# leodd/Lifted-Hybrid-Variational-Inference

Measured on AMD Instinct MI355X. Metric: lbp_sweeps_per_sec_10M_edge_hybrid_mrf, higher is better.
Workload: dtype f64

## Files before the change

include/lhvi.h:

```cpp
#ifndef LHVI_H
#define LHVI_H

#include <stddef.h>
#include <stdint.h>

#ifdef __cplusplus
extern "C" {
#endif

#define LHVI_ABI_VERSION 17
#define LHVI_MAX_ARITY 6

#define LHVI_OK 0
#define LHVI_E_ARG (-1)
#define LHVI_E_LAUNCH (-2)
#define LHVI_E_UNSUPPORTED (-3)
#define LHVI_E_NODEVICE (-4)
#define LHVI_E_NOT_PD (-5)

#define LHVI_POT_GENERIC 0
#define LHVI_POT_TABLE 1
#define LHVI_POT_GAUSSIAN 2
#define LHVI_POT_QUADRATIC 3
#define LHVI_POT_HYBRID_QUADRATIC 4
#define LHVI_POT_LINEAR_GAUSSIAN 5
#define LHVI_POT_X2 6
#define LHVI_POT_XY 7
#define LHVI_POT_MLN 8
#define LHVI_POT_MLN_HARD 9
#define LHVI_POT_IMAGE_NODE 10
#define LHVI_POT_IMAGE_EDGE 11

typedef struct lhvi_graph {
// ... 127 lines not shown
    const void* cq_desc;
    int32_t n_cq;
    const int32_t* v2f_wide;
    int32_t n_v2f_wide;
    const int32_t* v2f_narrow;
    int32_t n_v2f_narrow;
    const int32_t* v2f_hub;
    int32_t n_v2f_hub;
    const int32_t* v2f_mid16;
    int32_t n_v2f_mid16;
    const int32_t* v2f_mid32;
    int32_t n_v2f_mid32;
    const int32_t* prop_hub;
    int32_t n_prop_hub;
    double* prop_partial;
    const int32_t* resample_vars;
    int32_t n_resample_vars;
    const void* small16_desc;
    int32_t n_small16;
    const void* small32_desc;
    int32_t n_small32;
    const int64_t* halo_off;
    double* halo_buf;
} lhvi_pbp_t;

#define LHVI_PBP_DESC_BYTES 128
#define LHVI_PBP_TICKET_WORDS 16
#define LHVI_PBP_TICKET_COUNTERS 8
int lhvi_pbp_describe(const lhvi_graph_t* g, const lhvi_pots_t* pots, const lhvi_pbp_t* s, const int32_t* edges, int32_t count,
                      void* desc_out, void* stream);
int lhvi_pbp_describe_cq(const lhvi_graph_t* g, const lhvi_pots_t* pots, const lhvi_pbp_t* s, const int32_t* edges, int32_t count,
                         void* desc_out, void* stream);
int lhvi_pbp_var_sum(const lhvi_graph_t* g, const lhvi_pbp_t* s, const double* f2v, double* out, void* stream);
int lhvi_pbp_domain_grid(const lhvi_graph_t* g, const lhvi_pbp_t* s, double* x, void* stream);
int lhvi_pbp_refine_grid(const lhvi_graph_t* g, const lhvi_pbp_t* s, const double* logb, double* x, double* best, double* best_val,
                         void* stream);
int lhvi_debug_exp(const double* x, double* y, int64_t n, void* stream);
int lhvi_debug_exp_acc(const double* x, const double* c, double* y, int64_t n, void* stream);
int lhvi_debug_exp_acc_floor(const double* x, const double* c, double* y, int64_t n, void* stream);
int lhvi_debug_log(const double* x, double* y, int64_t n, int32_t which, void* stream);

int lhvi_pbp_classify(const lhvi_graph_t* g, const lhvi_pots_t* pots, const lhvi_pbp_t* s, uint8_t* edge_class, void* stream);

int lhvi_pbp_uniq(const lhvi_graph_t* g, int32_t n, const double* particles, const int32_t* np, uint8_t* uniq, void* stream);
int lhvi_pbp_v2f(const lhvi_graph_t* g, const lhvi_pbp_t* s, const double* f2v, double* v2f, void* stream);
int lhvi_pbp_f2v(const lhvi_graph_t* g, const lhvi_pots_t* pots, const lhvi_pbp_t* s, const double* v2f, double* f2v, void* stream);
// ... 207 lines not shown
```

lifted-hybrid-variational-inference_amd/csrc/fastmath.hpp:

```cpp
#pragma once
#include "common.hpp"

namespace lhvi {

#include "exp_table.inc"
constexpr int EXP_TAB_N = 1 << LHVI_EXP_TABLE_BITS;

__device__ __forceinline__ double exp_core(double t, const double* __restrict__ tab ) {
    const double MAGIC = LHVI_SCONST(6755399441055744.0);
    const double u = fma(t, LHVI_SCONST(LHVI_EXP_INV_STEP), MAGIC);
    const int nn = __double2loint(u);
    const double kd = u - MAGIC;
    double r = fma(kd, LHVI_SCONST(-LHVI_EXP_STEP_HI), t);
    r = fma(kd, LHVI_SCONST(-LHVI_EXP_STEP_LO), r);
    double p = fma(r, LHVI_SCONST(1.6666666666666666667e-1), 0.5);
    p = fma(p, r, 1.0);
    p = fma(p, r, 1.0);
    return ldexp(tab[nn & (EXP_TAB_N - 1)] * p, nn >> LHVI_EXP_TABLE_BITS);
}

__device__ __forceinline__ void load_exp_table(double* __restrict__ tab) {
    for (int i = threadIdx.x; i < EXP_TAB_N; i += blockDim.x) tab[i] = EXP_TAB[i];
    __syncthreads();
}
// ... 10 lines not shown
    double p = fma(r, 1.6666666666666666667e-1, 0.5);
    p = fma(p, r, 1.0);
    o.scale = fma(p, r, 1.0);
    return o;
}

__device__ __forceinline__ double exp_accumulate(double acc, double t, double magic, const double* __restrict__ tab) {
    double u;
    asm("v_fma_f64 %0, %1, %2, %3" : "=v"(u) : "v"(t), "s"((double)LHVI_EXP_INV_STEP), "v"(magic));
    const int nn = __double2loint(u);
    const double kd = u - magic;
    const double r = fma(kd, -LHVI_EXP_STEP_HI, t);
    double p = fma(r, 1.6666666666666666667e-1, 0.5);
    p = fma(p, r, 1.0);
    p = fma(p, r, 1.0);
    return fma(ldexp(tab[nn & (EXP_TAB_N - 1)], nn >> LHVI_EXP_TABLE_BITS), p, acc);
}

struct ExpShiftFloor { double magic, scale; };

__device__ __forceinline__ void round_down_on() { asm volatile("s_setreg_imm32_b32 hwreg(HW_REG_MODE, 2, 2), 2\n\ts_nop 1" ::: "memory"); }
__device__ __forceinline__ void round_down_off() { asm volatile("s_setreg_imm32_b32 hwreg(HW_REG_MODE, 2, 2), 0\n\ts_nop 1" ::: "memory"); }

__device__ __forceinline__ ExpShiftFloor exp_shift_floor(double C) {
    const double MAGIC = 6755399441055744.0;
    ExpShiftFloor o;
    const double m = fma(C, LHVI_EXP_INV_STEP, MAGIC);
    const double kd = m - MAGIC;
    double r = fma(kd, -LHVI_EXP_STEP_HI, C);
    r = fma(kd, -LHVI_EXP_STEP_LO, r);
    double p = fma(r, 1.6666666666666666667e-1, 0.5);
    p = fma(p, r, 1.0);
    o.scale = fma(p, r, 1.0) * LHVI_EXPF_SCALE;
    o.magic = 844424930131968.0 + (kd - (double)(24 << LHVI_EXP_TABLE_BITS));
    return o;
}

__device__ __forceinline__ double exp_accumulate_floor(double acc, double s, double magic, const double* __restrict__ tab) {
    double u;
    asm volatile("v_add_f64 %0, %1, %2" : "=v"(u) : "v"(s), "v"(magic));
    const int nn = __double2loint(u);
    const double f = __builtin_amdgcn_fract(s);
    double p = fma(f, LHVI_SCONST(LHVI_EXPF_RHO), 1.0);
    p = fma(p, f, LHVI_SCONST(LHVI_EXPF_K1));
    p = fma(p, f, LHVI_SCONST(LHVI_EXPF_K0));
    const double entry = *reinterpret_cast<const double*>(reinterpret_cast<const char*>(tab) + (nn & ((EXP_TAB_N - 1) << 3)));
    return fma(ldexp(entry, nn >> (LHVI_EXP_TABLE_BITS + 3)), p, acc);
}

constexpr int LOG_TAB_N = 1 << LHVI_LOG_TABLE_BITS;
struct LogRec { double inv_c, log_c; };

__device__ __forceinline__ void load_log_table(LogRec* __restrict__ tab) {
    for (int i = threadIdx.x; i < LOG_TAB_N; i += blockDim.x) { tab[i].inv_c = LOG_TAB[2 * i]; tab[i].log_c = LOG_TAB[2 * i + 1]; }
}

__device__ __forceinline__ double log_table(double x, const LogRec* __restrict__ tab) {
// ... 16 lines not shown
```

lifted-hybrid-variational-inference_amd/csrc/pbp.hip:

```cpp
#include "common.hpp"
#include "potential.hpp"
#include "fastmath.hpp"
#include "cq.hpp"

namespace lhvi {

__device__ __forceinline__ double wave_sum(double v) { return dpp_wave_reduce(v, SumOp()); }
__device__ __forceinline__ double wave_max(double v) { return dpp_wave_reduce(v, MaxOp()); }
__device__ __forceinline__ int wave_sum_i(int v) {
#pragma unroll
    for (int off = 32; off > 0; off >>= 1) v += __shfl_xor(v, off);
    return v;
}

constexpr double PAD_LOG_TERM = -6.0e5;

__host__ __device__ __forceinline__ int var_first(const lhvi_pbp_t& s) { return s.var_hi > s.var_lo ? s.var_lo : 0; }
__host__ __device__ __forceinline__ int var_limit(const lhvi_graph_t& g, const lhvi_pbp_t& s) { return s.var_hi > s.var_lo ? s.var_hi : g.V; }

__device__ __forceinline__ double norm_pdf_std(double x, double mu, double sig) {
    const double u = (x - mu) / sig;
    return exp(-u * u * 0.5) / (2.506628274631 * sig);
}

// ... 528 lines not shown
    double t;
    if (MODE == MODE_VARK) t = fma(shk[j], X2, fma(r.b, X1, r.a));
    else t = fma(r.b, fma(r.b, X2, X1), r.a);
    return exp_accumulate(acc, t, magic, tab);
}

template <int MODE>
__device__ __forceinline__ double fast_accumulate_uniform(const AB* __restrict__ sh, const double* __restrict__ shk,
                                                          const double* __restrict__ tab, int jn_, double X1, double X2, double C) {
    const int jn = __builtin_amdgcn_readfirstlane(jn_);
    const ExpShift sft = exp_shift(C);
    double acc0 = 0.0, acc1 = 0.0;
    int j = 0;
    for (; j + 2 <= jn; j += 2) {
        acc0 = fast_term<MODE>(acc0, sh, shk, tab, j, X1, X2, sft.magic);
        acc1 = fast_term<MODE>(acc1, sh, shk, tab, j + 1, X1, X2, sft.magic);
    }
    if (j < jn) acc0 = fast_term<MODE>(acc0, sh, shk, tab, j, X1, X2, sft.magic);
    return (acc0 + acc1) * sft.scale;
}

#define LHVI_PIN1(a) do { if (PIN) asm volatile("" : "+v"(a)); } while (0)
#define LHVI_PIN2(a, b) do { if (PIN) asm volatile("" : "+v"(a), "+v"(b)); } while (0)
template <int UNROLL = 4, bool PIN = false>
__device__ __forceinline__ double fast_accumulate_floor(const AB* __restrict__ sh, const double* __restrict__ tab, int jn_, double X1,
                                                        double C) {
    const int jn = __builtin_amdgcn_readfirstlane(jn_);
    LHVI_PIN1(C);
    ExpShiftFloor sft = exp_shift_floor(C);
    LHVI_PIN2(sft.magic, sft.scale);
    double acc0 = 0.0, acc1 = 0.0;
    int j = 0;
    round_down_on();
    if (UNROLL == 4) {
        double acc2 = 0.0, acc3 = 0.0;
        for (; j + 4 <= jn; j += 4) {
            const AB r0 = sh[j], r1 = sh[j + 1], r2 = sh[j + 2], r3 = sh[j + 3];
            acc0 = exp_accumulate_floor(acc0, fma(r0.b, X1, r0.a), sft.magic, tab);
            acc1 = exp_accumulate_floor(acc1, fma(r1.b, X1, r1.a), sft.magic, tab);
            acc2 = exp_accumulate_floor(acc2, fma(r2.b, X1, r2.a), sft.magic, tab);
            acc3 = exp_accumulate_floor(acc3, fma(r3.b, X1, r3.a), sft.magic, tab);
        }
        if (j < jn) { const AB r0 = sh[j]; acc0 = exp_accumulate_floor(acc0, fma(r0.b, X1, r0.a), sft.magic, tab); }
        if (j + 1 < jn) { const AB r1 = sh[j + 1]; acc1 = exp_accumulate_floor(acc1, fma(r1.b, X1, r1.a), sft.magic, tab); }
        if (j + 2 < jn) { const AB r2 = sh[j + 2]; acc2 = exp_accumulate_floor(acc2, fma(r2.b, X1, r2.a), sft.magic, tab); }
        acc0 += acc2; acc1 += acc3;
        LHVI_PIN2(acc0, acc1);
        round_down_off();
        return (acc0 + acc1) * sft.scale;
    }
    for (; j + 2 <= jn; j += 2) {
        const AB r0 = sh[j], r1 = sh[j + 1];
        acc0 = exp_accumulate_floor(acc0, fma(r0.b, X1, r0.a), sft.magic, tab);
        acc1 = exp_accumulate_floor(acc1, fma(r1.b, X1, r1.a), sft.magic, tab);
    }
    if (j < jn) { const AB r0 = sh[j]; acc0 = exp_accumulate_floor(acc0, fma(r0.b, X1, r0.a), sft.magic, tab); }
    LHVI_PIN2(acc0, acc1);
    round_down_off();
    return (acc0 + acc1) * sft.scale;
}

__global__ void __launch_bounds__(BLOCK) pbp_f2v_fast_kernel(lhvi_graph_t g, lhvi_pots_t pots, lhvi_pbp_t s,
                                                            const double* __restrict__ v2f, double* __restrict__ f2v,
                                                            const FastDesc* __restrict__ descs,
                                                            const double* __restrict__ param) {
    __shared__ AB sh_all[BLOCK / WAVE][WAVE];
    __shared__ double shk_all[BLOCK / WAVE][WAVE];
    __shared__ double sh_tab[EXP_TAB_N];
    __shared__ LogRec sh_log[LOG_TAB_N];
    load_log_table(sh_log);
    load_exp_table(sh_tab);
// ... 387 lines not shown
            }
        }
#pragma nounroll
        for (int r = 0; r < 2; ++r) {
            const int rem = npts - 64 * r;
            if (rem <= 0) break;
            const int lw = round_log2_width(rem);
            const int width = 1 << lw, split = 64 >> lw, sub = lane >> lw, pl = lane & (width - 1);
            const int p = 64 * r + pl;
            const bool valid = pl < rem;
            const double xv = r == 0 ? x0 : x1;
            const double X1 = valid ? xv : 0.0, C = kconst * X1 * X1;
            const int chunk = (s.flags & LHVI_PBP_SKIP_TERMS) ? 0 : (nj + split - 1) >> (6 - lw);
            double acc = fast_accumulate_floor<LHVI_HEAVY_UNROLL>(sh + sub * chunk, sh_tab, chunk, X1, C);
            for (int off = width; off < 64; off <<= 1) acc += __shfl_xor(acc, off);
            if (valid && sub == 0) out[p < np ? p : n + (p - np)] = acc > 0.0 ? log_table(acc, sh_log) : -700.0;
        }
        if (!more) break;
        cur.advance(nxt, lane);
    }
    if (stats && lane == 0) { atomicAdd(stats, (uint32_t)n_grid); atomicAdd(stats + 1, (uint32_t)n_direct); }
}

#ifndef LHVI_SMALL_WAVES
#define LHVI_SMALL_WAVES 6
#endif
#ifndef LHVI_SMALL_WAVES10
#define LHVI_SMALL_WAVES10 5
#endif
#ifndef LHVI_SMALL_WAVES2
#define LHVI_SMALL_WAVES2 5
#endif
template <int W, int PPL = 1>
__global__ void __launch_bounds__(BLOCK) __attribute__((amdgpu_waves_per_eu(PPL == 2 ? LHVI_SMALL_WAVES2 : W == 10 ? LHVI_SMALL_WAVES10 : LHVI_SMALL_WAVES, 8))) pbp_f2v_small_kernel(lhvi_graph_t g, lhvi_pbp_t s, const double* __restrict__ v2f,
                                                            double* __restrict__ f2v, const FastDesc* __restrict__ descs, int nitems) {
    using Geo = SmallGeom<W>;
    constexpr int G = Geo::G;
    constexpr int GS = PPL * W + 1;
    constexpr int SH_AB = G * GS > Geo::BUF_AB ? G * GS : Geo::BUF_AB;
    __shared__ AB sh_all[BLOCK / WAVE][SH_AB];
    __shared__ double sh_tab[EXP_TAB_N];
    __shared__ LogRec sh_log[LOG_TAB_N];
    load_log_table(sh_log);
    load_exp_table(sh_tab);
    const int wid = __builtin_amdgcn_readfirstlane(threadIdx.x >> 6);
    const int lane = threadIdx.x & 63;
// ... 1694 lines not shown
    hipLaunchKernelGGL(debug_exp_acc_floor_kernel, dim3(grid_for(n)), dim3(BLOCK), 0, as_stream(stream), x, c, y, n);
    return check_launch();
}

int lhvi_debug_exp_acc(const double* x, const double* c, double* y, int64_t n, void* stream) {
    if (!x || !c || !y || n < 0) return LHVI_E_ARG;
    if (n == 0) return LHVI_OK;
    hipLaunchKernelGGL(debug_exp_acc_kernel, dim3(grid_for(n)), dim3(BLOCK), 0, as_stream(stream), x, c, y, n);
    return check_launch();
}

int lhvi_pbp_v2f(const lhvi_graph_t* g, const lhvi_pbp_t* s, const double* f2v, double* v2f, void* stream) {
    if (int rc = validate_pbp(g, s)) return rc;
    if (!f2v || !v2f || !s->uniq || !s->q) return LHVI_E_ARG;
    if (s->halo_off && !s->halo_buf) return LHVI_E_ARG;
    if (g->V == 0) return LHVI_OK;
    return s->halo_off ? launch_v2f<true>(g, s, f2v, v2f, stream) : launch_v2f<false>(g, s, f2v, v2f, stream);
}

int lhvi_pbp_f2v(const lhvi_graph_t* g, const lhvi_pots_t* pots, const lhvi_pbp_t* s, const double* v2f, double* f2v, void* stream) {
    if (int rc = validate_pbp(g, s)) return rc;
    if (!pots || !v2f || !f2v || !s->old_particles) return LHVI_E_ARG;
    if ((s->flags & LHVI_PBP_CQ) && (!s->fast_edges || !s->generic_edges)) return LHVI_E_ARG;
    if (s->n_small16 < 0 || s->n_small32 < 0 || (s->n_small16 > 0 && !s->small16_desc) || (s->n_small32 > 0 && !s->small32_desc)) return LHVI_E_ARG;
    if (g->E == 0) return LHVI_OK;
    const int nfast = s->fast_edges ? s->n_fast : g->E, ngen = s->generic_edges ? s->n_generic : g->E;
    static const int cus = device_cus();
    static const int fast_per_cu = blocks_per_cu((const void*)pbp_f2v_fast_kernel);
    static const int heavy_per_cu = blocks_per_cu((const void*)pbp_f2v_heavy_kernel, HEAVY_BLOCK);
    static const int light_per_cu = blocks_per_cu((const void*)pbp_f2v_light_kernel);
    static const int gen_per_cu = blocks_per_cu((const void*)pbp_f2v_generic_kernel<true>);
    static const int gen_slim_per_cu = blocks_per_cu((const void*)pbp_f2v_generic_kernel<false>);
    const int share = (s->flags & LHVI_PBP_SHARE_CUS) ? 1 : 0;
    const int spare = (s->flags & LHVI_PBP_LEAVE_ROOM) ? max(cus / 8, 1) : 0;
    auto short_grid = [&](int items, int per_cu) { return dim3(min((items + 3) / 4, max(cus * min(per_cu, 8) - spare, 1))); };
    const uint32_t families = s->flags & LHVI_PBP_F2V_ALL;
    auto want = [families](uint32_t family) { return families == 0 || (families & family) != 0; };
    if (want(LHVI_PBP_F2V_HEAVY) && s->heavy_desc && s->n_heavy > 0) {
        constexpr int HWPB = HEAVY_BLOCK / WAVE;
        const int heavy_grid = min((s->n_heavy + HWPB - 1) / HWPB, max(cus * max(heavy_per_cu - share, 1) - spare * (BLOCK / WAVE) / HWPB, 1));
        lhvi_pbp_t sh = *s;
        if (sh.f2v_ticket && (int64_t)s->n_heavy < (int64_t)heavy_grid * HWPB * 8 * 4) sh.f2v_ticket = nullptr;
        if (s->f2v_ticket && hipMemsetAsync(s->f2v_ticket, 0, LHVI_PBP_TICKET_WORDS * sizeof(uint32_t), as_stream(stream)) != hipSuccess)
            return LHVI_E_LAUNCH;
        hipLaunchKernelGGL(pbp_f2v_heavy_kernel, dim3(heavy_grid), dim3(HEAVY_BLOCK), 0, as_stream(stream),
                           *g, sh, v2f, f2v, reinterpret_cast<const FastDesc*>(s->heavy_desc), s->n_heavy,
                           s->f2v_ticket ? s->f2v_ticket + LHVI_PBP_TICKET_COUNTERS : (uint32_t*)nullptr);
    }
    if (want(LHVI_PBP_F2V_SMALL)) {
        const bool narrow = !(s->flags & LHVI_PBP_POW2_GROUPS);
        if (s->small16_desc && s->n_small16 > 0) {
            if (narrow && s->n <= 10) launch_f2v_small<10>(g, s, v2f, f2v, s->small16_desc, s->n_small16, cus, share, spare, stream);
            else if (narrow && s->n <= 12) launch_f2v_small<6, 2>(g, s, v2f, f2v, s->small16_desc, s->n_small16, cus, share, spare, stream);
            else if (narrow) launch_f2v_small<8, 2>(g, s, v2f, f2v, s->small16_desc, s->n_small16, cus, share, spare, stream);
            else launch_f2v_small<16>(g, s, v2f, f2v, s->small16_desc, s->n_small16, cus, share, spare, stream);
        }
        if (s->small32_desc && s->n_small32 > 0) {
            if (narrow && s->n <= 20) launch_f2v_small<10, 2>(g, s, v2f, f2v, s->small32_desc, s->n_small32, cus, share, spare, stream);
            else if (narrow && s->n <= 24) launch_f2v_small<12, 2>(g, s, v2f, f2v, s->small32_desc, s->n_small32, cus, share, spare, stream);
            else if (narrow) launch_f2v_small<16, 2>(g, s, v2f, f2v, s->small32_desc, s->n_small32, cus, share, spare, stream);
            else launch_f2v_small<32>(g, s, v2f, f2v, s->small32_desc, s->n_small32, cus, share, spare, stream);
        }
    }
    if (want(LHVI_PBP_F2V_PAIR)) {
        if (s->pair_desc && s->n_pair > 0 && !(s->flags & LHVI_PBP_WIDE_PAIRS) && s->n <= 32) {
            const bool narrow_pairs = !(s->flags & LHVI_PBP_POW2_GROUPS);
            if (s->n <= 16) launch_f2v_pair_small<16>(g, s, v2f, f2v, cus, spare, stream);
            else if (narrow_pairs && s->n <= 20) launch_f2v_pair_small<20>(g, s, v2f, f2v, cus, spare, stream);
            else launch_f2v_pair_small<32>(g, s, v2f, f2v, cus, spare, stream);
        } else if (s->pair_desc && s->n_pair > 0) {
            static const int pair_per_cu = blocks_per_cu((const void*)pbp_f2v_pair_kernel);
// ... 250 lines not shown
```

lifted-hybrid-variational-inference_amd/lhvi/_abi.py:

```python
from __future__ import annotations

import ctypes as C
import os

import numpy as np

_HERE = os.path.dirname(os.path.abspath(__file__))
LIB_PATH = os.environ.get('LHVI_LIB') or os.path.join(os.path.dirname(_HERE), 'csrc', 'liblhvi.so')

c_i32p = C.c_void_p
c_f64p = C.c_void_p


class LhviError(RuntimeError):
    pass


class GraphStruct(C.Structure):
    _fields_ = [
        ('V', C.c_int32), ('F', C.c_int32), ('E', C.c_int32), ('nnz', C.c_int32),
        ('fac_ptr', C.c_void_p), ('edge_var', C.c_void_p), ('edge_fac', C.c_void_p), ('edge_canon', C.c_void_p),
        ('var_ptr', C.c_void_p), ('var_edge', C.c_void_p), ('edge_count', C.c_void_p), ('fac_pot', C.c_void_p),
        ('var_value', C.c_void_p), ('var_dom', C.c_void_p), ('var_mult', C.c_void_p), ('fac_mult', C.c_void_p),
        ('D', C.c_int32),
# ... 13 lines not shown

class PbpStruct(C.Structure):
    _fields_ = [
        ('n', C.c_int32), ('T', C.c_int32), ('flags', C.c_uint32),
        ('var_threshold', C.c_double), ('max_log_value', C.c_double),
        ('particles', C.c_void_p), ('old_particles', C.c_void_p), ('np', C.c_void_p), ('uniq', C.c_void_p),
        ('q', C.c_void_p),
        ('fast_edges', C.c_void_p), ('n_fast', C.c_int32), ('generic_edges', C.c_void_p), ('n_generic', C.c_int32),
        ('generic_pts_log2', C.c_int32), ('fast_desc', C.c_void_p), ('heavy_desc', C.c_void_p), ('n_heavy', C.c_int32), ('light_desc', C.c_void_p), ('n_light', C.c_int32),
        ('bslot', C.c_void_p), ('brow_ptr', C.c_void_p), ('brow_off', C.c_void_p), ('brow_peer', C.c_void_p),
        ('recv', C.c_void_p), ('rank', C.c_int32), ('var_degree', C.c_void_p),
        ('var_lo', C.c_int32), ('var_hi', C.c_int32),
        ('f2v_ticket', C.c_void_p),
        ('prop_desc', C.c_void_p), ('n_prop_desc', C.c_int32),
        ('pair_desc', C.c_void_p), ('n_pair', C.c_int32),
        ('cq_desc', C.c_void_p), ('n_cq', C.c_int32),
        ('v2f_wide', C.c_void_p), ('n_v2f_wide', C.c_int32), ('v2f_narrow', C.c_void_p), ('n_v2f_narrow', C.c_int32),
        ('v2f_hub', C.c_void_p), ('n_v2f_hub', C.c_int32),
        ('v2f_mid16', C.c_void_p), ('n_v2f_mid16', C.c_int32), ('v2f_mid32', C.c_void_p), ('n_v2f_mid32', C.c_int32),
        ('prop_hub', C.c_void_p), ('n_prop_hub', C.c_int32), ('prop_partial', C.c_void_p),
        ('resample_vars', C.c_void_p), ('n_resample_vars', C.c_int32),
        ('small16_desc', C.c_void_p), ('n_small16', C.c_int32), ('small32_desc', C.c_void_p), ('n_small32', C.c_int32),
        ('halo_off', C.c_void_p), ('halo_buf', C.c_void_p),
    ]


class ViStruct(C.Structure):
    _fields_ = [
        ('K', C.c_int32), ('T', C.c_int32), ('Dmax', C.c_int32), ('quirks', C.c_int32),
        ('gh_x', C.c_void_p), ('gh_w', C.c_void_p), ('w', C.c_void_p), ('eta_c', C.c_void_p), ('eta_d', C.c_void_p),
        ('obs_var', C.c_void_p), ('var_N', C.c_void_p),
        ('fac_list', C.c_void_p), ('n_cc', C.c_int32), ('n_grp3', C.c_int32), ('n_grp6', C.c_int32), ('n_rest3', C.c_int32),
        ('n_rest6', C.c_int32), ('n_tiny', C.c_int32), ('tiny_par_words', C.c_int32), ('edge_axis', C.c_void_p),
    ]


class ViOptStruct(C.Structure):
    _fields_ = [(n, C.c_void_p) for n in ('w_tau', 'w', 'eta_c', 'tau_d', 'eta_d', 'm_w', 's_w', 'm_c', 's_c', 'm_d', 's_d',
                                          'g_w', 'g_c', 'g_d', 'fe')] + \
               [(n, C.c_double) for n in ('lr', 'b1', 'b2', 'eps', 'var_min')] + [('t', C.c_int32)]


PBP_EP = 1
PBP_EPBP_DISCRETE = 2
PBP_SKIP_TERMS = 16
PBP_NO_GRID = 128
PBP_LEAVE_ROOM = 256
PBP_BOUNDARY_TOTALS = 2048
PBP_CQ = 512
PBP_NO_UNIQ = 4096
PBP_V2F_RECORDS = 8192
PBP_WIDE_PAIRS = 16384
PBP_SHARE_CUS = 32768
PBP_POW2_GROUPS = 65536
PBP_FUSED_RECORDS16 = 131072
PBP_F2V_HEAVY = 262144
PBP_F2V_SMALL = 524288
PBP_F2V_PAIR = 1048576
PBP_F2V_FAST = 2097152
PBP_F2V_CQ = 4194304
PBP_F2V_GENERIC = 8388608
PBP_F2V_ALL = PBP_F2V_HEAVY | PBP_F2V_SMALL | PBP_F2V_PAIR | PBP_F2V_FAST | PBP_F2V_CQ | PBP_F2V_GENERIC
ABI_VERSION = 17
PBP_DESC_BYTES = 128
COLOR_HASH, COLOR_SORT = 0, 1
HUB_DEGREE = 64
VI_GROUP_SLOTS, VI_GROUP_COMP, VI_TINY_NODES, VI_TINY_K, VI_TINY_PAR = 24, 48, 32, 2, 3072

class MwsStruct(C.Structure):
    _fields_ = [('T', C.c_int32), ('max_flips', C.c_int32), ('epsilon', C.c_double), ('noise_std', C.c_double),
                ('seed', C.c_uint64), ('try_id', C.c_void_p), ('disc', C.c_void_p), ('n_disc', C.c_int32),
                ('num', C.c_void_p), ('n_num', C.c_int32), ('fac_class', C.c_void_p), ('x', C.c_void_p), ('best_x', C.c_void_p),
                ('cur_score', C.c_void_p), ('best_score', C.c_void_p), ('status', C.c_void_p), ('err_flip', C.c_void_p),
                ('rec_score', C.c_void_p), ('rec_zero', C.c_void_p), ('rec_ticks', C.c_void_p)] + \
               [(n, C.c_void_p) for n in ('rp_init', 'rp_clause', 'rp_walk', 'rp_walk_k', 'rp_noise', 'rp_post', 'out_score',
                                          'out_unsat', 'out_winner', 'out_accept', 'out_val')]


class ExactStruct(C.Structure):
    _fields_ = [('Nd', C.c_int32), ('Nc', C.c_int32), ('M', C.c_int64), ('dstates', C.c_void_p), ('dstride', C.c_void_p),
                ('n_quad', C.c_int32), ('quad_ptr', C.c_void_p), ('quad_desc', C.c_void_p), ('quad_par', C.c_void_p),
                ('n_tab', C.c_int32), ('tab_ptr', C.c_void_p), ('tab_desc', C.c_void_p), ('tab_par', C.c_void_p)]


class GibbsStruct(C.Structure):
    _fields_ = [('ex', ExactStruct), ('dstate_off', C.c_void_p), ('vt_ptr', C.c_void_p), ('vt_fac', C.c_void_p),
# ... 286 lines not shown
```

lifted-hybrid-variational-inference_amd/lhvi/pbp.py:

```python
from __future__ import annotations

import os
from math import e, log, sqrt

import numpy as np

from . import _abi
from .flat import flatten

_F2V_LONG = _abi.PBP_F2V_HEAVY | _abi.PBP_F2V_SMALL
_F2V_SHORT = _abi.PBP_F2V_PAIR | _abi.PBP_F2V_FAST | _abi.PBP_F2V_CQ | _abi.PBP_F2V_GENERIC
F2V_SCHEDULES = {
    'one': (('main', _abi.PBP_F2V_ALL, 0, False),),
    'timed': (('main', _F2V_LONG, 0, True), ('main', _F2V_SHORT, 0, False)),
    'overlap': (('side', _F2V_SHORT, 0, False), ('main', _F2V_LONG, _abi.PBP_SHARE_CUS, True)),
}


class _ParticleSweep:
    var_threshold = 3
    max_log_value = 700
    _epbp_discrete = True
    verbose = False
    listed_proposal = True
    dynamic_f2v = True
    paired_light = True
    cq_routing = True
    small_f2v = True
    long_grid_min_edges = 1 << 16
    listed_resample = True
    sliced_proposal = True
    prop_slice = 64
    packed_v2f = True
    overlap_f2v = True
    overlap_min_heavy = 1 << 16
    fused_var_kernel = True
    fused_max_particles = 32
    exact_queries = False
    map_mode = 'fminbound'

    def _setup(self, graph_like, flat=None, edge_key=None, sides='vf', edge_skip=None, owned=None):
        flat = flat if flat is not None else flatten(graph_like, require_device_potentials=True)
        self.flat = flat
        self.dg = dg = _abi.DeviceGraph(flat)
        torch = _abi.require_gpu()
        n = self.n
        sizes = np.diff(flat.dom_ptr)
        cont = flat.dom_cont.astype(bool)
        self.T = int(sizes[cont].max()) if cont.any() else 0
        nst = flat.var_nstates
        if (flat.var_hidden & ~flat.var_cont & (nst > n)).any():
# ... 107 lines not shown
                    vs = vs[~fused_var[vs]]
                    host_lists['v2f_rest_' + name] = (self._v2f_records(flat, vs) if name == 'wide' and os.environ.get('LHVI_PBP_V2F_REC', '1') != '0' else
                                                      vs.astype(np.int32) if vs.size else np.zeros(1, dtype=np.int32))
                    rest_parts.append((name, int(vs.size)))
            self._fused = dict(counts=(int(k16.sum()), int(k32a.sum()), int(k32b.sum())), n_prop_rest=int(keep.sum()),
                               n_resample_rest=int(rkeep.sum()), rest_parts=rest_parts)
        dev_lists = _abi.upload(host_lists)
        for name in ('np_dev', 'resample_vars', '_static_idx', 'prop_desc'):
            setattr(self, name, dev_lists[name])
        if self._fused is not None:
            F = self._fused
            F['desc'], F['prop_desc_rest'], F['resample_rest'] = dev_lists['fused_desc'], dev_lists['prop_desc_rest'], dev_lists['resample_rest']
            F['v2f_rest'] = tuple(x for name, cnt in F['rest_parts'] for x in (dev_lists['v2f_rest_' + name], cnt)) if F['rest_parts'] else None
        if 'prop_hub' in dev_lists:
            self.prop_hub = dev_lists['prop_hub']
        if 'v2f_wide' in dev_lists:
            self.v2f_lists = tuple(x for name, m in parts for x in (dev_lists['v2f_' + name], int(m.sum())))
            if os.environ.get('LHVI_PBP_V2F_REC', '1') != '0':
                self.flags |= _abi.PBP_V2F_RECORDS
        pad = torch.zeros(1, dtype=torch.int32, device=dg.device)
        self.cq_edges = pad[:0]
        self.part_counts = {'heavy': 0, 'light': 0, 'fast': 0, 'generic': 0, 'cq': 0, 'pair': 0, 'small16': 0, 'small32': 0}
        self.generic_pts_log2 = 6
        self.fast_desc = self.heavy_desc = self.light_desc = self.pair_desc = self.small16_desc = self.small32_desc = None
        self.n_heavy = self.n_light = self.n_pair = self.n_small16 = self.n_small32 = self.n_heavy_class = 0
        self.cq_terms = self.heavy_terms = self.heavy_grid_terms = 0
        self._has_f_side = 'f' in sides
        if not self._has_f_side:
            self.fast_edges = self.generic_edges = pad[:0]
            self._fast_list = self._generic_list = pad
            return
        cls = torch.zeros(max(flat.E, 1), dtype=torch.uint8, device=dg.device)
        _abi.check(_abi.lib().lhvi_pbp_classify(dg.g, dg.p, self._struct(), _abi.ptr(cls), _abi.stream_ptr()))
        cls = cls[:flat.E]
        if edge_skip is not None:
            cls = torch.where(_abi.to_dev(np.ascontiguousarray(edge_skip, dtype=bool)), torch.zeros_like(cls), cls)
        self.fast_edges = torch.nonzero((cls == 1) | (cls == 2)).flatten().to(torch.int32)
        self.generic_edges = torch.nonzero(cls == 3).flatten().to(torch.int32)
        self.cq_edges = torch.nonzero(cls == 4).flatten().to(torch.int32)
        key_dev = None
        if edge_key is not None:
            key_dev = _abi.to_dev(np.ascontiguousarray(edge_key, dtype=np.int32))
            self.fast_edges = self.fast_edges[torch.sort(key_dev[self.fast_edges.long()], stable=True).indices].contiguous()
            self.generic_edges = self.generic_edges[torch.sort(key_dev[self.generic_edges.long()], stable=True).indices].contiguous()
            self.cq_edges = self.cq_edges[torch.sort(key_dev[self.cq_edges.long()], stable=True).indices].contiguous()

        def first_part(edges):
# ... 15 lines not shown
            cw = cqd.view(torch.int32).view(ncq, 2 * _abi.PBP_DESC_BYTES // 4).to(torch.int64)
            self.cq_terms = int(torch.where(cw[:, 2] == 1, (cw[:, 4] + cw[:, 5]) * cw[:, 9] * cw[:, 3],
                                            cw[:, 3] * cw[:, 12] * cw[:, 9]).sum().item())
        nf = int(self.fast_edges.numel())
        if nf:
            desc = torch.empty(nf * _abi.PBP_DESC_BYTES, dtype=torch.uint8, device=dg.device)
            _abi.check(_abi.lib().lhvi_pbp_describe(dg.g, dg.p, self._struct(), _abi.ptr(self.fast_edges), nf,
                                                    _abi.ptr(desc), _abi.stream_ptr()))
            words = desc.view(torch.int32).view(nf, _abi.PBP_DESC_BYTES // 4)
            base = (words[:, 4] == 1) & (words[:, 6] != 4)
            small16 = small32 = torch.zeros_like(base)
            if self.small_f2v:
                small16 = base & (words[:, 7] <= 16) & (words[:, 8] <= 16)
                small32 = base & ~small16 & (words[:, 7] <= 32) & (words[:, 8] <= 32)
            small = small16 | small32
            on_recurrence = (words[:, 15] == 1) & (words[:, 7] >= 24) & (words[:, 9] <= 128) & (words[:, 8] <= 128)
            two_rounds = words[:, 8] + words[:, 9] <= 128
            if int((on_recurrence & ~two_rounds & ~small).sum().item()) < self.long_grid_min_edges:
                on_recurrence = two_rounds
            heavy = (base & (words[:, 7] <= 64) & (two_rounds | on_recurrence)) | small
            rows = desc.view(nf, _abi.PBP_DESC_BYTES)
            self.small16_desc, self.small32_desc = rows[small16].contiguous(), rows[small32].contiguous()
            self.n_small16, self.n_small32 = int(self.small16_desc.shape[0]), int(self.small32_desc.shape[0])
            self.n_heavy_class = int(heavy.sum().item())
            self.heavy_desc = rows[heavy & ~small].contiguous()
            self.n_heavy = int(self.heavy_desc.shape[0])
            hw = words[heavy].to(torch.int64)
            self.heavy_terms = int(((hw[:, 8] + hw[:, 9]) * hw[:, 7]).sum().item())
            on_grid = (hw[:, 15] == 1) & (hw[:, 9] <= 128) & ((hw[:, 7] >= 24) | small[heavy])
            self.heavy_grid_terms = int((hw[:, 9] * hw[:, 7])[on_grid].sum().item())
            light = ~heavy & (words[:, 14] != 0)
            self.light_desc = rows[light].contiguous()
            self.n_light = int(self.light_desc.shape[0])
            rest = ~heavy & ~light
            self.fast_desc = rows[rest].contiguous()
            all_fast = self.fast_edges
            self.fast_edges = all_fast[rest].contiguous()
            self._fast_list = self.fast_edges if self.fast_edges.numel() else pad
            self.part_counts.update(heavy=first_part(all_fast[heavy & ~small]), light=first_part(all_fast[light]),
                                    fast=first_part(self.fast_edges), small16=first_part(all_fast[small16]),
                                    small32=first_part(all_fast[small32]))
            self._build_pairs(key_dev)

    def _v2f_records(self, flat, vs):
        rec = np.zeros((max(int(vs.size), 1), 8), dtype=np.int32)
        if vs.size:
            deg = np.diff(flat.var_ptr)[vs]
            rec[:, 0], rec[:, 1], rec[:, 2], rec[:, 3] = vs, deg, self.np_host[vs], flat.var_dom[vs]
            base = flat.var_ptr[vs].astype(np.int64)
            for k in range(4):
                if flat.var_edge.size:
                    rec[:, 4 + k] = flat.var_edge[np.minimum(base + np.minimum(k, np.maximum(deg - 1, 0)), flat.var_edge.size - 1)]
        return rec

    def _build_pairs(self, key_dev):
        torch = _abi.require_gpu()
        if not self.paired_light or self.light_desc is None or self.n_light == 0:
            return
        dev = self.light_desc.device
        w = self.light_desc.view(torch.int32).view(-1, 32).long()
        dd = self.light_desc.view(torch.float64).view(-1, 16)
        i1, i2 = torch.nonzero(w[:, 14] == 1).flatten(), torch.nonzero(w[:, 14] == 2).flatten()
# ... 28 lines not shown
            od[n1:, 6:12] = rd[:, 8:14]
            ow[n1:, 25] = r2[:, 3].int()
        first = 0
        if key_dev is not None and n1 + n2:
            edge = torch.where(ow[:, 0] >= 0, ow[:, 0], ow[:, 1]).long()
            order = torch.sort(key_dev[edge], stable=True).indices
            out = out[order].contiguous()
            first = int((key_dev[edge] == 0).sum().item())
        self.pair_desc, self.n_pair = out, n1 + n2
        self.part_counts['pair'] = first

    def _struct(self):
        s = _abi.PbpStruct()
        s.n, s.T, s.flags = self.n, self.T, self.flags
        s.var_threshold, s.max_log_value = float(self.var_threshold), float(self.max_log_value)
        s.particles, s.old_particles = _abi.ptr(self.particles), _abi.ptr(self.old_particles)
        s.np, s.uniq, s.q = _abi.ptr(self.np_dev), _abi.ptr(self.uniq), _abi.ptr(self.q_dev)
        s.fast_edges, s.n_fast = _abi.ptr(self._fast_list), int(self.fast_edges.numel())
        s.generic_edges, s.n_generic = _abi.ptr(self._generic_list), int(self.generic_edges.numel())
        s.generic_pts_log2 = int(getattr(self, 'generic_pts_log2', 6))
        s.fast_desc = _abi.ptr(getattr(self, 'fast_desc', None))
        s.heavy_desc, s.n_heavy = _abi.ptr(getattr(self, 'heavy_desc', None)), int(getattr(self, 'n_heavy', 0))
        s.light_desc, s.n_light = _abi.ptr(getattr(self, 'light_desc', None)), int(getattr(self, 'n_light', 0))
        if getattr(self, 'n_small16', 0):
            s.small16_desc, s.n_small16 = _abi.ptr(self.small16_desc), int(self.n_small16)
        if getattr(self, 'n_small32', 0):
            s.small32_desc, s.n_small32 = _abi.ptr(self.small32_desc), int(self.n_small32)
        if self.paired_light and getattr(self, 'pair_desc', None) is not None:
            s.pair_desc, s.n_pair = _abi.ptr(self.pair_desc), int(self.n_pair)
        s.cq_desc, s.n_cq = _abi.ptr(getattr(self, 'cq_desc', None)), int(getattr(self, 'n_cq', 0))
        if getattr(self, 'v2f_lists', None) is not None:
            w, nw, nr, nn, hb, nh, m16, n16, m32, n32 = self.v2f_lists
            s.v2f_wide, s.n_v2f_wide, s.v2f_narrow, s.n_v2f_narrow = _abi.ptr(w), nw, _abi.ptr(nr), nn
            s.v2f_hub, s.n_v2f_hub = _abi.ptr(hb), nh
            s.v2f_mid16, s.n_v2f_mid16, s.v2f_mid32, s.n_v2f_mid32 = _abi.ptr(m16), n16, _abi.ptr(m32), n32
        s.f2v_ticket = _abi.ptr(self.f2v_ticket) if self.dynamic_f2v else None
        if self.listed_proposal and getattr(self, 'prop_desc', None) is not None:
            s.prop_desc, s.n_prop_desc = _abi.ptr(self.prop_desc), self.n_prop_desc
            if getattr(self, 'prop_hub', None) is not None:
                s.prop_hub, s.n_prop_hub, s.prop_partial = _abi.ptr(self.prop_hub), self.n_prop_hub, _abi.ptr(self.prop_partial)
        return s

    def _host_draw(self):
        flat = self.flat
        q = self.q_dev.cpu().numpy()
        out = np.zeros((flat.V, self.n))
# ... 935 lines not shown
```

Baseline: 66.00.

## Route single-term heavy f2v edges to a dedicated paired-wave kernel

Heavy factor-to-variable edges whose sum has only one term (words[7]==1, pval defined, not small or few) are split out of the heavy list into a new oneterm kernel. In that kernel each wave processes two edges, with the next pair's descriptors and particles prefetched while the current pair is computed. The general heavy path's reduction and unroll overhead is skipped for these edges. The floor-exp shift is also split into pieces so the polynomial scale is computed after the accumulation loop, which eases register pressure. This adds a new ABI field, a new launch and partition logic, with some risk of mismatched classification or numerical drift.

```diff
diff --git a/include/lhvi.h b/include/lhvi.h
--- a/include/lhvi.h
+++ b/include/lhvi.h
@@ -8,7 +8,7 @@
 extern "C" {
 #endif
 
-#define LHVI_ABI_VERSION 17
+#define LHVI_ABI_VERSION 18
 #define LHVI_MAX_ARITY 6
 
 #define LHVI_OK 0
@@ -182,6 +182,8 @@
     int32_t n_small32;
     const int64_t* halo_off;
     double* halo_buf;
+    const void* oneterm_desc;
+    int32_t n_oneterm;
 } lhvi_pbp_t;
 
 #define LHVI_PBP_DESC_BYTES 128
diff --git a/lifted-hybrid-variational-inference_amd/csrc/fastmath.hpp b/lifted-hybrid-variational-inference_amd/csrc/fastmath.hpp
--- a/lifted-hybrid-variational-inference_amd/csrc/fastmath.hpp
+++ b/lifted-hybrid-variational-inference_amd/csrc/fastmath.hpp
@@ -56,17 +56,27 @@
 __device__ __forceinline__ void round_down_on() { asm volatile("s_setreg_imm32_b32 hwreg(HW_REG_MODE, 2, 2), 2\n\ts_nop 1" ::: "memory"); }
 __device__ __forceinline__ void round_down_off() { asm volatile("s_setreg_imm32_b32 hwreg(HW_REG_MODE, 2, 2), 0\n\ts_nop 1" ::: "memory"); }
 
-__device__ __forceinline__ ExpShiftFloor exp_shift_floor(double C) {
+__device__ __forceinline__ double exp_shift_floor_k(double C) {
     const double MAGIC = 6755399441055744.0;
-    ExpShiftFloor o;
     const double m = fma(C, LHVI_EXP_INV_STEP, MAGIC);
-    const double kd = m - MAGIC;
+    return m - MAGIC;
+}
+__device__ __forceinline__ double exp_shift_floor_magic(double kd) {
+    return 844424930131968.0 + (kd - (double)(24 << LHVI_EXP_TABLE_BITS));
+}
+__device__ __forceinline__ double exp_shift_floor_poly(double kd, double C) {
     double r = fma(kd, -LHVI_EXP_STEP_HI, C);
     r = fma(kd, -LHVI_EXP_STEP_LO, r);
     double p = fma(r, 1.6666666666666666667e-1, 0.5);
     p = fma(p, r, 1.0);
-    o.scale = fma(p, r, 1.0) * LHVI_EXPF_SCALE;
-    o.magic = 844424930131968.0 + (kd - (double)(24 << LHVI_EXP_TABLE_BITS));
+    return fma(p, r, 1.0);
+}
+
+__device__ __forceinline__ ExpShiftFloor exp_shift_floor(double C) {
+    ExpShiftFloor o;
+    const double kd = exp_shift_floor_k(C);
+    o.scale = exp_shift_floor_poly(kd, C) * LHVI_EXPF_SCALE;
+    o.magic = exp_shift_floor_magic(kd);
     return o;
 }
 
diff --git a/lifted-hybrid-variational-inference_amd/csrc/pbp.hip b/lifted-hybrid-variational-inference_amd/csrc/pbp.hip
--- a/lifted-hybrid-variational-inference_amd/csrc/pbp.hip
+++ b/lifted-hybrid-variational-inference_amd/csrc/pbp.hip
@@ -574,16 +574,27 @@
 
 #define LHVI_PIN1(a) do { if (PIN) asm volatile("" : "+v"(a)); } while (0)
 #define LHVI_PIN2(a, b) do { if (PIN) asm volatile("" : "+v"(a), "+v"(b)); } while (0)
-template <int UNROLL = 4, bool PIN = false>
+template <int UNROLL = 4, int PIN = 0>
 __device__ __forceinline__ double fast_accumulate_floor(const AB* __restrict__ sh, const double* __restrict__ tab, int jn_, double X1,
                                                         double C) {
+    static_assert(PIN != 2 || UNROLL == 4, "PIN == 2 reproduces the heavy kernel, which runs the loop unrolled by four");
     const int jn = __builtin_amdgcn_readfirstlane(jn_);
     LHVI_PIN1(C);
-    ExpShiftFloor sft = exp_shift_floor(C);
-    LHVI_PIN2(sft.magic, sft.scale);
+    ExpShiftFloor sft;
+    double kd = 0.0, poly = 0.0;
+    if (PIN == 2) {
+        kd = exp_shift_floor_k(C);
+        sft.magic = exp_shift_floor_magic(kd);
+        sft.scale = 0.0;
+        asm volatile("" : "+v"(kd), "+v"(sft.magic));
+    } else {
+        sft = exp_shift_floor(C);
+        LHVI_PIN2(sft.magic, sft.scale);
+    }
     double acc0 = 0.0, acc1 = 0.0;
     int j = 0;
     round_down_on();
+    if (PIN == 2) asm volatile("" : "+v"(kd));
     if (UNROLL == 4) {
         double acc2 = 0.0, acc3 = 0.0;
         for (; j + 4 <= jn; j += 4) {
@@ -597,8 +608,13 @@
         if (j + 1 < jn) { const AB r1 = sh[j + 1]; acc1 = exp_accumulate_floor(acc1, fma(r1.b, X1, r1.a), sft.magic, tab); }
         if (j + 2 < jn) { const AB r2 = sh[j + 2]; acc2 = exp_accumulate_floor(acc2, fma(r2.b, X1, r2.a), sft.magic, tab); }
         acc0 += acc2; acc1 += acc3;
+        if (PIN == 2) { poly = exp_shift_floor_poly(kd, C); asm volatile("" : "+v"(poly)); }
         LHVI_PIN2(acc0, acc1);
         round_down_off();
+        if (PIN == 2) {
+            asm volatile("" : "+v"(poly), "+v"(acc0), "+v"(acc1));
+            sft.scale = poly * LHVI_EXPF_SCALE;
+        }
         return (acc0 + acc1) * sft.scale;
     }
     for (; j + 2 <= jn; j += 2) {
@@ -1032,6 +1048,112 @@
     if (stats && lane == 0) { atomicAdd(stats, (uint32_t)n_grid); atomicAdd(stats + 1, (uint32_t)n_direct); }
 }
 
+struct OneTermEdge { int32_t e, tv, np, T, gb; double kx; };
+struct OneTermData { double xa, xb, xg; };
+
+__device__ __forceinline__ OneTermEdge oneterm_edge(const FastDesc& d, bool live) {
+    OneTermEdge o;
+    o.e = d.e; o.tv = d.tv; o.np = live ? d.np : 0; o.T = live ? d.T : 0; o.gb = d.gb; o.kx = d.kx;
+    return o;
+}
+__device__ __forceinline__ AB oneterm_record(const FastDesc& d) {
+    const double y = d.pval;
+    AB r;
+    r.a = (fma(fma(d.ay, y, d.by), y, d.c) + 0.0) * LHVI_EXP_INV_STEP;
+    r.b = fma(d.axy, y, d.bx) * LHVI_EXP_INV_STEP;
+    return r;
+}
+__device__ __forceinline__ OneTermData oneterm_fetch(const OneTermEdge& A, const OneTermEdge& B, const double* __restrict__ particles,
+                                                     const double* __restrict__ dom_val, int n, int lane) {
+    OneTermData h;
+    h.xa = 0.0; h.xb = 0.0; h.xg = 0.0;
+    if (lane < A.np) h.xa = particles[(int64_t)A.tv * n + lane];
+    if (lane < B.np) h.xb = particles[(int64_t)B.tv * n + lane];
+    const int t = lane & 31;
+    if (t < (lane < 32 ? A.T : B.T)) h.xg = dom_val[(lane < 32 ? A.gb : B.gb) + t];
+    return h;
+}
+__device__ __forceinline__ double oneterm_point(const AB* __restrict__ rec, const double* __restrict__ tab, const LogRec* __restrict__ logtab,
+                                                double x, double kx, bool valid) {
+    const double X1 = valid ? x : 0.0, C = kx * X1 * X1;
+    const double acc = fast_accumulate_floor<4, 2>(rec, tab, 1, X1, C);
+    return acc > 0.0 ? log_table(acc, logtab) : -700.0;
+}
+
+__global__ void __launch_bounds__(BLOCK) pbp_f2v_oneterm_kernel(const double* __restrict__ particles, const double* __restrict__ dom_val,
+                                                               double* __restrict__ f2v, const FastDesc* __restrict__ descs,
+                                                               int nitems, int n, int S) {
+    __shared__ AB sh_all[BLOCK / WAVE][2];
+    __shared__ double sh_tab[EXP_TAB_N];
+    __shared__ LogRec sh_log[LOG_TAB_N];
+    load_log_table(sh_log);
+    load_exp_table(sh_tab);
+    const int wid = __builtin_amdgcn_readfirstlane(threadIdx.x >> 6);
+    const int lane = threadIdx.x & 63;
+    AB* sh = sh_all[wid];
+    const int npairs = (nitems + 1) >> 1, last = nitems - 1;
+    const int nwaves = gridDim.x * (BLOCK / WAVE);
+    int pair = blockIdx.x * (BLOCK / WAVE) + wid;
+    if (pair >= npairs) return;
+    FastDesc dA = descs[2 * pair], dB = descs[min(2 * pair + 1, last)];
+    OneTermEdge A = oneterm_edge(dA, true), B = oneterm_edge(dB, 2 * pair + 1 <= last);
+    OneTermData h = oneterm_fetch(A, B, particles, dom_val, n, lane);
+    AB recA = oneterm_record(dA), recB = oneterm_record(dB);
+    for (;;) {
+        const int nxt = pair + nwaves;
+        const bool more = nxt < npairs;
+        const int ia = __builtin_amdgcn_readfirstlane(min(2 * nxt, last)), ib = __builtin_amdgcn_readfirstlane(min(2 * nxt + 1, last));
+        dA = descs[ia]; dB = descs[ib];
+        LHVI_WAVE_SYNC();
+        if (lane < 2) {
+            AB r;
+            r.a = lane ? recB.a : recA.a; r.b = lane ? recB.b : recA.b;
+            sh[lane] = r;
+        }
+        LHVI_WAVE_SYNC();
+        const OneTermEdge cA = A, cB = B;
+        const OneTermData c = h;
+        if (more) {
+            A = oneterm_edge(dA, true); B = oneterm_edge(dB, 2 * nxt + 1 <= last);
+            recA = oneterm_record(dA); recB = oneterm_record(dB);
+            h = oneterm_fetch(A, B, particles, dom_val, n, lane);
+        }
+#pragma nounroll
+        for (int k = 0; k < 2; ++k) {
+            const int np = k ? cB.np : cA.np, tv = k ? cB.tv : cA.tv;
+            const double kx = k ? cB.kx : cA.kx;
+            double* out = f2v + (int64_t)(k ? cB.e : cA.e) * S;
+#pragma nounroll
+            for (int p0 = 0; p0 < np; p0 += 64) {
+                const int pp = p0 + lane;
+                const bool valid = pp < np;
+                double x = k ? c.xb : c.xa;
+                if (p0) { x = 0.0; if (valid) x = particles[(int64_t)tv * n + pp]; }
+                const double v = oneterm_point(sh + k, sh_tab, sh_log, x, kx, valid);
+                if (valid) out[pp] = v;
+            }
+        }
+        {
+            const bool hi = lane >= 32;
+            const int t1 = lane & 31, T = hi ? cB.T : cA.T, gb = hi ? cB.gb : cA.gb, Tmax = max(cA.T, cB.T);
+            const double kx = hi ? cB.kx : cA.kx;
+            double* out = f2v + (int64_t)(hi ? cB.e : cA.e) * S + n;
+            const AB* rec = sh + (hi ? 1 : 0);
+#pragma nounroll
+            for (int t0 = 0; t0 < Tmax; t0 += 32) {
+                const int t = t0 + t1;
+                const bool valid = t < T;
+                double x = c.xg;
+                if (t0) { x = 0.0; if (valid) x = dom_val[gb + t]; }
+                const double v = oneterm_point(rec, sh_tab, sh_log, x, kx, valid);
+                if (valid) out[t] = v;
+            }
+        }
+        if (!more) break;
+        pair = nxt;
+    }
+}
+
 #ifndef LHVI_SMALL_WAVES
 #define LHVI_SMALL_WAVES 6
 #endif
@@ -2772,6 +2894,7 @@
     if (int rc = validate_pbp(g, s)) return rc;
     if (!pots || !v2f || !f2v || !s->old_particles) return LHVI_E_ARG;
     if ((s->flags & LHVI_PBP_CQ) && (!s->fast_edges || !s->generic_edges)) return LHVI_E_ARG;
+    if (s->n_oneterm < 0 || (s->n_oneterm > 0 && !s->oneterm_desc)) return LHVI_E_ARG;
     if (s->n_small16 < 0 || s->n_small32 < 0 || (s->n_small16 > 0 && !s->small16_desc) || (s->n_small32 > 0 && !s->small32_desc)) return LHVI_E_ARG;
     if (g->E == 0) return LHVI_OK;
     const int nfast = s->fast_edges ? s->n_fast : g->E, ngen = s->generic_edges ? s->n_generic : g->E;
@@ -2797,6 +2920,11 @@
                            *g, sh, v2f, f2v, reinterpret_cast<const FastDesc*>(s->heavy_desc), s->n_heavy,
                            s->f2v_ticket ? s->f2v_ticket + LHVI_PBP_TICKET_COUNTERS : (uint32_t*)nullptr);
     }
+    if (want(LHVI_PBP_F2V_PAIR) && s->oneterm_desc && s->n_oneterm > 0) {
+        static const int oneterm_per_cu = blocks_per_cu((const void*)pbp_f2v_oneterm_kernel);
+        hipLaunchKernelGGL(pbp_f2v_oneterm_kernel, short_grid((s->n_oneterm + 1) / 2, oneterm_per_cu), dim3(BLOCK), 0, as_stream(stream),
+                           s->particles, g->dom_val, f2v, reinterpret_cast<const FastDesc*>(s->oneterm_desc), s->n_oneterm, s->n, s->n + s->T);
+    }
     if (want(LHVI_PBP_F2V_SMALL)) {
         const bool narrow = !(s->flags & LHVI_PBP_POW2_GROUPS);
         if (s->small16_desc && s->n_small16 > 0) {
diff --git a/lifted-hybrid-variational-inference_amd/lhvi/_abi.py b/lifted-hybrid-variational-inference_amd/lhvi/_abi.py
--- a/lifted-hybrid-variational-inference_amd/lhvi/_abi.py
+++ b/lifted-hybrid-variational-inference_amd/lhvi/_abi.py
@@ -59,6 +59,7 @@
         ('resample_vars', C.c_void_p), ('n_resample_vars', C.c_int32),
         ('small16_desc', C.c_void_p), ('n_small16', C.c_int32), ('small32_desc', C.c_void_p), ('n_small32', C.c_int32),
         ('halo_off', C.c_void_p), ('halo_buf', C.c_void_p),
+        ('oneterm_desc', C.c_void_p), ('n_oneterm', C.c_int32),
     ]
 
 
@@ -98,7 +99,7 @@
 PBP_F2V_CQ = 4194304
 PBP_F2V_GENERIC = 8388608
 PBP_F2V_ALL = PBP_F2V_HEAVY | PBP_F2V_SMALL | PBP_F2V_PAIR | PBP_F2V_FAST | PBP_F2V_CQ | PBP_F2V_GENERIC
-ABI_VERSION = 17
+ABI_VERSION = 18
 PBP_DESC_BYTES = 128
 COLOR_HASH, COLOR_SORT = 0, 1
 HUB_DEGREE = 64
diff --git a/lifted-hybrid-variational-inference_amd/lhvi/pbp.py b/lifted-hybrid-variational-inference_amd/lhvi/pbp.py
--- a/lifted-hybrid-variational-inference_amd/lhvi/pbp.py
+++ b/lifted-hybrid-variational-inference_amd/lhvi/pbp.py
@@ -27,6 +27,7 @@
     paired_light = True
     cq_routing = True
     small_f2v = True
+    oneterm_f2v = True
     long_grid_min_edges = 1 << 16
     listed_resample = True
     sliced_proposal = True
@@ -180,7 +181,8 @@
         self.cq_edges = pad[:0]
         self.part_counts = {'heavy': 0, 'light': 0, 'fast': 0, 'generic': 0, 'cq': 0, 'pair': 0, 'small16': 0, 'small32': 0}
         self.generic_pts_log2 = 6
-        self.fast_desc = self.heavy_desc = self.light_desc = self.pair_desc = self.small16_desc = self.small32_desc = None
+        self.fast_desc = self.heavy_desc = self.light_desc = self.pair_desc = self.small16_desc = self.small32_desc = self.oneterm_desc = None
+        self.n_oneterm = 0
         self.n_heavy = self.n_light = self.n_pair = self.n_small16 = self.n_small32 = self.n_heavy_class = 0
         self.cq_terms = self.heavy_terms = self.heavy_grid_terms = 0
         self._has_f_side = 'f' in sides
@@ -242,6 +244,14 @@
             rows = desc.view(nf, _abi.PBP_DESC_BYTES)
             self.small16_desc, self.small32_desc = rows[small16].contiguous(), rows[small32].contiguous()
             self.n_small16, self.n_small32 = int(self.small16_desc.shape[0]), int(self.small32_desc.shape[0])
+            oneterm = torch.zeros_like(base)
+            if self.oneterm_f2v and edge_key is None and os.environ.get('LHVI_PBP_ONETERM', '1') != '0':
+                pval = desc.view(torch.float64).view(nf, _abi.PBP_DESC_BYTES // 8)[:, 6]
+                few = (words[:, 7] <= 32) & (words[:, 8] <= 32)
+                oneterm = heavy & ~small & ~few & (words[:, 7] == 1) & ~torch.isnan(pval)
+            self.oneterm_desc = rows[oneterm].contiguous()
+            self.n_oneterm = int(self.oneterm_desc.shape[0])
+            heavy = heavy & ~oneterm
             self.n_heavy_class = int(heavy.sum().item())
             self.heavy_desc = rows[heavy & ~small].contiguous()
             self.n_heavy = int(self.heavy_desc.shape[0])
@@ -249,6 +259,7 @@
             self.heavy_terms = int(((hw[:, 8] + hw[:, 9]) * hw[:, 7]).sum().item())
             on_grid = (hw[:, 15] == 1) & (hw[:, 9] <= 128) & ((hw[:, 7] >= 24) | small[heavy])
             self.heavy_grid_terms = int((hw[:, 9] * hw[:, 7])[on_grid].sum().item())
+            heavy = heavy | oneterm
             light = ~heavy & (words[:, 14] != 0)
             self.light_desc = rows[light].contiguous()
             self.n_light = int(self.light_desc.shape[0])
@@ -257,7 +268,7 @@
             all_fast = self.fast_edges
             self.fast_edges = all_fast[rest].contiguous()
             self._fast_list = self.fast_edges if self.fast_edges.numel() else pad
-            self.part_counts.update(heavy=first_part(all_fast[heavy & ~small]), light=first_part(all_fast[light]),
+            self.part_counts.update(heavy=first_part(all_fast[heavy & ~small & ~oneterm]), light=first_part(all_fast[light]),
                                     fast=first_part(self.fast_edges), small16=first_part(all_fast[small16]),
                                     small32=first_part(all_fast[small32]))
             self._build_pairs(key_dev)
@@ -332,6 +343,8 @@
         s.fast_desc = _abi.ptr(getattr(self, 'fast_desc', None))
         s.heavy_desc, s.n_heavy = _abi.ptr(getattr(self, 'heavy_desc', None)), int(getattr(self, 'n_heavy', 0))
         s.light_desc, s.n_light = _abi.ptr(getattr(self, 'light_desc', None)), int(getattr(self, 'n_light', 0))
+        if getattr(self, 'n_oneterm', 0):
+            s.oneterm_desc, s.n_oneterm = _abi.ptr(self.oneterm_desc), int(self.n_oneterm)
         if getattr(self, 'n_small16', 0):
             s.small16_desc, s.n_small16 = _abi.ptr(self.small16_desc), int(self.n_small16)
         if getattr(self, 'n_small32', 0):
```

Measured after the change: 65.48. Within noise of the previous version (-0.8%).
